# abiswas-odu/metagenomics

Measured on AMD Instinct MI355X. Metric: overlap edges/sec, higher is better.
Workload: dtype u64

## Files before the change

metagenomics_amd/csrc/device/mg_ctx.hpp:

```cpp
#ifndef MG_CTX_HPP_
#define MG_CTX_HPP_
#include <hip/hip_runtime.h>

#include <algorithm>
#include <cstdint>
#include <string>
#include <vector>

#include "mg_overlap.h"

__host__ __device__ constexpr int slot_words(int w) {
  return w <= 1 ? 1 : w <= 2 ? 2 : w <= 4 ? 4 : w <= 8 ? 8 : w <= 16 ? 16 : 32;
}

__host__ __device__ constexpr int slot_id_word(int w) { return slot_words(w) >= w + 2 ? slot_words(w) - 1 : -1; }
static_assert(slot_id_word(5) == 7 && slot_id_word(6) == 7 && slot_id_word(12) == 15, "widths with a spare word");
static_assert(slot_id_word(1) == -1 && slot_id_word(2) == -1 && slot_id_word(3) == -1 && slot_id_word(4) == -1 &&
                  slot_id_word(8) == -1 && slot_id_word(16) == -1 && slot_id_word(32) == -1,
              "widths whose slot ends at the pad word (or before it)");

template <typename T>
struct DevArray {
  T* p = nullptr;
  size_t cap = 0;
// ... 199 lines not shown
  uint8_t* xmarks = nullptr;
  uint64_t xchg_lo = 0, xchg_hi = 0;
  unsigned long long* d_blk = nullptr;
  size_t blk_cap = 0;
  unsigned long long* d_rcnt = nullptr;
  size_t rcnt_cap = 0;
  uint8_t* d_rdst = nullptr;
  size_t rdst_cap = 0;
  bool runs_meta8 = false;
  uint64_t super_zero_n = 0;
  unsigned long long* d_kblk = nullptr;
  size_t kblk_cap = 0;
  bool keys_counted = false;
  bool runs_counted = false;
  bool index_times_pending = false;
  unsigned long long* d_dcnt = nullptr;
  size_t dcnt_cap = 0;
  bool rows_counted = false;
  bool xchg_route_rows = true;
  bool xchg_scan_lds = true;
  uint32_t xchg_region = 512;
  uint32_t xchg_split_max = 4;
  int packable = 0;
  unsigned long long* d_flat_cnt = nullptr;
  size_t flat_cnt_cap = 0;
  unsigned long long* d_slot_cnt = nullptr;
  size_t slot_cnt_cap = 0;
  uint32_t* d_kb = nullptr;
  uint64_t* d_ke = nullptr;
  size_t kb_cap = 0, ke_cap = 0;
  hipEvent_t ev[16] = {};
  int scan_state = 0;
  bool runs_live = false;
  bool probe_share = true;
  bool probe_compact = true;
  uint64_t* d_key0 = nullptr;
  size_t key0_cap = 0;
  bool prefix_probe = true;
  ulonglong2* d_p0runs = nullptr;
  size_t p0runs_cap = 0;
  unsigned long long* d_p0cnt = nullptr;
  size_t p0cnt_cap = 0;
  uint32_t* d_xk[2] = {nullptr, nullptr};
  ulonglong2* d_xv[2] = {nullptr, nullptr};
  size_t xk_cap[2] = {0, 0}, xv_cap[2] = {0, 0};
  void* d_xsort_tmp = nullptr;
  size_t xsort_tmp_cap = 0;
  int xv_sel = 0;
  uint64_t xruns_n = 0;
  bool own_probed = false;
  bool xchg_keys_first = true;
  bool keys_first = false;
  bool rk_on = false;
  const uint64_t* rk_keys = nullptr;
  const unsigned long long* rk_cnt = nullptr;
  uint64_t rk_slot = 0, rk_total = 0;
  int xruns_part = 0;
  uint64_t xruns_K = 0;
  ulonglong2* d_xexp = nullptr;
  size_t xexp_cap = 0;
  bool xruns_ready = false;
  ulonglong2* xruns_base = nullptr;
  unsigned long long* xruns_cnt = nullptr;
  uint64_t xruns_reg = 0, xruns_nreg = 0;
  uint32_t* d_xkk[2] = {nullptr, nullptr};
  uint64_t* d_xke[2] = {nullptr, nullptr};
// ... 152 lines not shown
```

metagenomics_amd/csrc/device/mg_kernels.hip:

```cpp
#include <hip/hip_runtime.h>

#include <hipcub/hipcub.hpp>

#include <algorithm>
#include <cmath>
#include <cstdint>
#include <cstring>
#include <string>
#include <vector>

#include "mg_ctx.hpp"
#include "mg_overlap.h"

#ifndef MG_SCAN_UNROLL
#define MG_SCAN_UNROLL 1
#endif

namespace {

constexpr int kWave = 64;
constexpr int kBlock = 256;
constexpr int kWavesPerBlock = kBlock / kWave;
constexpr int kSegs = 64;
constexpr uint32_t kFpBits = 9;

__device__ __forceinline__ uint64_t mix64(uint64_t x) {
  x ^= x >> 31;
  x *= 0x7fb5d329728ea185ULL;
  x ^= x >> 27;
  x *= 0x81dadef4bc2dd44dULL;
  x ^= x >> 33;
  return x;
}

__device__ __forceinline__ uint32_t order_key(uint64_t mm) {
  const uint32_t lo = (uint32_t)mm, hi = (uint32_t)(mm >> 32);
  uint32_t x = __umul24(lo, 0x9E3779u) + (hi ^ (lo >> 8));
  x ^= x >> 15;
  x = __umul24(x, 0xEBCA77u) + (x >> 8);
  x ^= x >> 13;
  return x & 0xFFFFFC00u;
}

__device__ __forceinline__ uint64_t rc_word(uint64_t x) {
  x = __builtin_bitreverse64(~x);
// ... 611 lines not shown
  uint32_t recv_P;
  uint8_t* run_dst;
};

__device__ __forceinline__ int key_seg(int o) { return o == 0 ? 0 : (o == 1 ? 3 : o - 1); }

__device__ __forceinline__ void wave_sync() {
  __builtin_amdgcn_fence(__ATOMIC_RELEASE, "wavefront");
  __builtin_amdgcn_wave_barrier();
  __builtin_amdgcn_fence(__ATOMIC_ACQUIRE, "wavefront");
}

__device__ __forceinline__ uint64_t run_meta(uint64_t a, int p, int jlo, int jhi) {
  return (a & 0xFFFFFFFFull) | ((uint64_t)p << 32) | ((uint64_t)jlo << 42) | ((uint64_t)jhi << 52);
}


template <int MAXW>
__device__ __forceinline__ uint64_t ext_reg(const uint64_t* rw, int pos) {
  const int wi = pos >> 5;
  uint64_t w0 = rw[0], w1 = rw[1];
#pragma unroll
  for (int k = 1; k <= MAXW; ++k) {
    w0 = wi == k ? rw[k] : w0;
    w1 = wi + 1 == k ? rw[k] : w1;
  }
  if (wi + 1 > MAXW) w1 = 0;
  return funnel(w0, w1, (pos & 31) << 1);
}

#ifndef MG_SCAN_WAVES_G
#define MG_SCAN_WAVES_G 6
#endif
template <int MAXW, bool INDEX, bool KEYREC = false, int G = 1, bool RECV = false>
__global__ __launch_bounds__(kBlock) __attribute__((amdgpu_waves_per_eu(G > 1 ? MG_SCAN_WAVES_G : 6))) void k_scan(ScanParams p) {
  extern __shared__ __attribute__((aligned(16))) uint64_t smem[];
  const int lane = threadIdx.x & 63, wv = threadIdx.x >> 6;
  const int h = p.h, m = p.m, w = p.w;
  uint32_t* s_keys = reinterpret_cast<uint32_t*>(smem) + (size_t)wv * (w + kScanKeyPad) * kWave + lane;
  const int msh = 64 - 2 * m;
  const uint64_t mmask = (m == 32) ? ~0ULL : ((1ULL << (2 * m)) - 1);
  const uint64_t ngroups = (p.a_hi - p.a_lo + kWave - 1) / kWave;
  const int wpb = (int)(blockDim.x >> 6);
  const uint64_t gw = (uint64_t)blockIdx.x * wpb + wv;
  const uint64_t nw = (uint64_t)gridDim.x * wpb;
  uint64_t* s_buf = reinterpret_cast<uint64_t*>(smem) + (size_t)wpb * (((w + kScanKeyPad) * kWave + 1) / 2) +
                    (size_t)wv * kScanBuf;
  s_keys[w * kWave] = 0xFFFFFFFFu;
  ulonglong2* const region = p.runs + gw * G * p.run_cap;
  const uint64_t nbmask = (1ULL << p.nb_log2) - 1;
  uint64_t cur[G] = {};
  uint32_t dcnt = 0;
  uint32_t nbuf = 0;

  auto put = [&](bool flag, uint64_t meta) {
    const uint64_t bal = __ballot(flag);
    uint32_t at = nbuf + lane_prefix(bal);
    __asm__ volatile("" : "+v"(at));
    s_buf[flag ? at : 2 * kWave + lane] = meta;
    nbuf += (uint32_t)__popcll(bal);
  };
  const uint64_t nwin = (ngroups + G - 1) / G;
  uint64_t r_at = 0, r_end = 0, r_per = 0;
  if constexpr (RECV) {
    const uint64_t nch = (p.recv_total + 63) / 64;
    const uint64_t ch0 = nch * gw / nw, ch1 = nch * (gw + 1) / nw;
    r_at = ch0 * 64;
    r_end = min(ch1 * 64, p.recv_total);
// ... 38 lines not shown
   if (G > 1 && __builtin_amdgcn_readfirstlane(lmin) != __builtin_amdgcn_readfirstlane(lmax)) {
#pragma unroll
     for (int k = 2; k <= G * kWave; k <<= 1) {
#pragma unroll
       for (int j = k >> 1; j > 0; j >>= 1) {
#pragma unroll
         for (int q = 0; q < G; ++q) {
           const int e = lane + kWave * q;
           const bool up = (e & k) == 0;
           if (j >= kWave) {
             const int q2 = q ^ (j / kWave);
             if (q < q2) {
               const uint32_t x = wk[q], y = wk[q2];
               const bool sw = up ? x > y : x < y;
               wk[q] = sw ? y : x;
               wk[q2] = sw ? x : y;
             }
           } else {
             const uint32_t o = (uint32_t)__shfl_xor((int)wk[q], j);
             const bool low = (e & j) == 0;
             wk[q] = (low == up) ? min(wk[q], o) : max(wk[q], o);
           }
         }
       }
     }
   }
   for (int q = 0; q < G; ++q) {
    uint32_t key = wk[0];
#pragma unroll
    for (int qq = 1; qq < G; ++qq) key = q == qq ? wk[qq] : key;
    const uint32_t wslot = key & 255u;
    const uint64_t a = A0 + wslot;
    const int n = (int)(0x7FFu - (key >> 8));
    const uint64_t own = G > 1 ? ((uint64_t)lane << 8) | wslot : a;
    const uint64_t* g = p.words + a * slot_words(MAXW);
    const int J = n - h - 1;
    const int tend = J >= 1 ? J + w - 1 : 0;
    const int tlast = (INDEX && tend) ? tend + 1 : tend;
    int tmax = tlast;
#pragma unroll
    for (int d = 32; d >= 1; d >>= 1) tmax = max(tmax, __shfl_xor(tmax, d));
    tmax = __builtin_amdgcn_readfirstlane(tmax);
    constexpr int kRw = MAXW + 1 <= slot_words(MAXW) ? MAXW + 1 : slot_words(MAXW);
    uint64_t rw[MAXW + 1];
    {
      const uint64_t* gs = a < p.a_hi ? g : p.words;
#pragma unroll
      for (int k = 0; k <= MAXW; ++k) rw[k] = k < kRw ? gs[k] : 0;
    }
    __builtin_amdgcn_s_waitcnt(kWaitVm0);
    auto word_at = [&](int idx) {
      uint64_t v = rw[0];
#pragma unroll
      for (int k = 1; k <= MAXW; ++k) v = idx == k ? rw[k] : v;
      return v;
    };
    auto flush = [&](uint32_t k) {
      wave_sync();
      bool flag = (uint32_t)lane < k;
      uint64_t v = 0, meta = 0;
      if (flag) meta = s_buf[lane];
      const uint32_t ws = G > 1 ? (uint32_t)meta & 255u : (uint32_t)meta - (uint32_t)A0;
      if (G > 1) meta = (meta & ~0xFFFFFFFFull) | (uint32_t)(A0 + ws);
      if constexpr (MAXW <= 8) {
        const int pos = (int)((meta >> 32) & 1023u), wi = pos >> 5;
        const int src = !flag ? lane : G > 1 ? (int)((uint32_t)s_buf[lane] >> 8 & 63u) : (int)ws;
        uint64_t w0 = 0, w1 = 0;
  #pragma unroll
        for (int kk = 0; kk <= MAXW; ++kk) {
          const uint32_t lo = (uint32_t)__builtin_amdgcn_ds_bpermute(src << 2, (int)(uint32_t)rw[kk]);
          const uint32_t hi = (uint32_t)__builtin_amdgcn_ds_bpermute(src << 2, (int)(uint32_t)(rw[kk] >> 32));
          const uint64_t x = ((uint64_t)hi << 32) | lo;
          w0 = wi == kk ? x : w0;
          w1 = wi + 1 == kk ? x : w1;
        }
        if (flag) {
          v = mix64(funnel(w0, w1, (pos & 31) << 1) >> msh);
          if (!INDEX || p.nranks > 1) flag = owned(v & nbmask, p.nb_log2, p.rank, p.nranks);
        }
      } else if (flag) {
        const uint64_t* g2 = p.words + (meta & 0xFFFFFFFFull) * slot_words(MAXW);
        const int pos = (int)((meta >> 32) & 1023u);
        v = mix64(funnel(g2[pos >> 5], g2[(pos >> 5) + 1], (pos & 31) << 1) >> msh);
        if (!INDEX || p.nranks > 1) flag = owned(v & nbmask, p.nb_log2, p.rank, p.nranks);
      }
      uint64_t at_rec = 0;
      uint32_t grp_rec = 0;
      if constexpr (G == 1) {
        const uint64_t bal = __ballot(flag);
        const uint64_t at = cur[0] + lane_prefix(bal);
        at_rec = at;
        if constexpr (RECV) {
          if (flag && at < p.run_cap) {
            reinterpret_cast<uint64_t*>(p.runs)[gw * p.run_cap + at] = meta;
            p.run_dst[gw * p.run_cap + at] = (uint8_t)(((v & nbmask) * p.dst_ranks) >> p.nb_log2);
          }
        } else {
#if defined(MG_DIAG_STORE_NEVER)
        if (flag && at < p.run_cap && v == 0x0123456789ABCDEFull) region[at] = make_ulonglong2(v, meta);
#elif !defined(MG_DIAG_NO_RUNSTORE)
        if (flag && at < p.run_cap) region[at] = make_ulonglong2(v, meta);
#endif
        }
        cur[0] += (uint64_t)__popcll(bal);
      } else {
#ifdef MG_DIAG_ONE_REGION
        const uint32_t grp = 0;
#else
        const uint32_t grp = ws >> 6;
#endif
        uint64_t at = 0;
#pragma unroll
        for (int j = 0; j < G; ++j) {
          const uint64_t bal = __ballot(flag && grp == (uint32_t)j);
          if (grp == (uint32_t)j) at = cur[j] + lane_prefix(bal);
          cur[j] += (uint64_t)__popcll(bal);
        }
        at_rec = at;
        grp_rec = grp;
#if defined(MG_DIAG_STORE_NEVER)
        if (flag && at < p.run_cap && v == 0x0123456789ABCDEFull) region[grp * p.run_cap + at] = make_ulonglong2(v, meta);
#elif !defined(MG_DIAG_NO_RUNSTORE)
        if (flag && at < p.run_cap) region[grp * p.run_cap + at] = make_ulonglong2(v, meta);
#endif
      }
      if constexpr (KEYREC || RECV) {
        if (p.dst_cnt) {
          const bool st = flag && at_rec < p.run_cap;
          const uint32_t d = st ? (uint32_t)(((v & nbmask) * p.dst_ranks) >> p.nb_log2) : 0u;
          for (uint32_t jj = 0; jj < (uint32_t)G; ++jj)
            for (uint32_t dd = 0; dd < p.dst_ranks; ++dd) {
              const uint32_t cc = (uint32_t)__popcll(__ballot(st && grp_rec == jj && d == dd));
              dcnt += (uint32_t)lane == jj * p.dst_ranks + dd ? cc : 0u;
            }
        }
      }
      const uint32_t rest = nbuf - k;
      const uint64_t m0 = (uint32_t)lane < rest ? s_buf[k + lane] : 0;
      const uint64_t m1 = (uint32_t)lane + kWave < rest ? s_buf[k + kWave + lane] : 0;
      wave_sync();
      if ((uint32_t)lane < rest) s_buf[lane] = m0;
      if ((uint32_t)lane + kWave < rest) s_buf[kWave + lane] = m1;
      nbuf = rest;
      wave_sync();
      __builtin_amdgcn_s_waitcnt(0xC07F);
    };
    uint64_t mm = 0;
    if (tend) mm = funnel(rw[0], rw[1], 2) >> msh;
    uint32_t kb0 = 0xFFFFFFFFu, kb1 = 0xFFFFFFFFu;
    if (INDEX && tend) kb0 = order_key(rw[0] >> msh);
    uint32_t pmin = 0xFFFFFFFFu;
    int last_pos = 0, jlo = 1;
    int u = 0;
    uint32_t sv_pf = s_keys[kWave];
    auto roll_and_advance = [&](uint32_t key, uint64_t cw, int sh) {
      s_keys[u * kWave] = key;
      mm = ((mm << 2) | ((cw >> sh) & 3u)) & mmask;
      if (++u == w) {
        uint32_t run = 0xFFFFFFFFu;
        for (int v0 = w - 1; v0 >= 0; v0 -= 8) {
          uint32_t x8[8];
#pragma unroll
          for (int k = 0; k < 8; ++k) x8[k] = v0 - k >= 0 ? s_keys[(v0 - k) * kWave] : 0xFFFFFFFFu;
#pragma unroll
          for (int k = 0; k < 8; ++k) {
            run = x8[k] < run ? x8[k] : run;
            if (v0 - k >= 0) s_keys[(v0 - k) * kWave] = run;
          }
        }
        u = 0;
        pmin = 0xFFFFFFFFu;
      }
      sv_pf = s_keys[(u + 1) * kWave];
    };
    auto step_first = [&](int t, uint64_t cw, int sh) {
      const uint32_t key = order_key(mm) | (uint32_t)t;
      pmin = min(pmin, key);
      if (INDEX && t == w - 1) kb0 = min(kb0, pmin);
      if (t == w) last_pos = (int)(min(sv_pf, pmin) & 1023u);
      roll_and_advance(key, cw, sh);
    };
    auto step = [&](int t, uint64_t cw, int sh) {
      const uint32_t key = order_key(mm) | (uint32_t)t;
      pmin = min(pmin, key);
      const uint32_t mn = min(sv_pf, pmin);
      const int pos = (int)(mn & 1023u);
      if (INDEX) kb1 = t == tlast ? mn - (uint32_t)(n - h) : kb1;
      const bool live = t <= tend;
      const bool emit = live && pos != last_pos;
      const uint64_t e_meta = run_meta(own, last_pos, jlo, t - w);
      jlo = emit ? t - w + 1 : jlo;
      last_pos = live ? pos : last_pos;
      roll_and_advance(key, cw, sh);
      put(emit, e_meta);
      if (nbuf >= (uint32_t)kWave) flush(kWave);
    };
    if constexpr (MAXW <= 8) {
#pragma unroll
      for (int k = 0; k < MAXW + (INDEX ? 1 : 0); ++k) {
        const int t0 = max(1, 32 * k - m), t1 = min(tmax, 32 * k + 31 - m);
        const int tf = min(t1, w);
        for (int t = t0, sh = 62 - 2 * ((t0 + m) & 31); t <= tf; ++t, sh -= 2) step_first(t, rw[k], sh);
        int t = max(t0, w + 1), sh = 62 - 2 * ((t + m) & 31);
        if (t <= t1) {
#if MG_SCAN_UNROLL == 2
          for (; t + 1 <= t1; t += 2, sh -= 4) {
            step(t, rw[k], sh);
            step(t + 1, rw[k], sh - 2);
          }
          if (t <= t1) step(t, rw[k], sh);
#else
          do {
            step(t, rw[k], sh);
            sh -= 2;
          } while (++t <= t1);
#endif
        }
      }
    } else {
      int cwi = __builtin_amdgcn_readfirstlane((1 + m) >> 5);
      uint64_t cw = word_at(cwi);
      for (int t = 1; t <= tmax; ++t) {
        const int sh = 62 - 2 * ((t + m) & 31);
        if (t <= w) step_first(t, cw, sh); else step(t, cw, sh);
        const int xu = __builtin_amdgcn_readfirstlane(t + m);
        if ((xu & 31) == 31) cw = word_at((xu + 1) >> 5);
      }
    }
    put(tend > 0, run_meta(own, last_pos, jlo, J));
    while (nbuf) flush(nbuf < (uint32_t)kWave ? nbuf : (uint32_t)kWave);
    if (INDEX && tend) {
      uint32_t kb2 = 0xFFFFFFFFu, kb3 = 0xFFFFFFFFu;
      const bool w32 = w <= 32;
      if (w32) {
        const uint64_t Aw = ext_reg<MAXW>(rw, n - h);
        uint64_t r3 = rc_word(funnel(rw[0], rw[1], 2 * (w - 1))) & mmask;
        uint64_t r2 = rc_word(ext_reg<MAXW>(rw, n - m)) & mmask;
        for (int i = 0; i < w; ++i) {
          kb3 = min(kb3, order_key(r3) | (uint32_t)i);
          kb2 = min(kb2, order_key(r2) | (uint32_t)i);
          const int t3 = w - 2 - i;
          if (t3 >= 0) {
            r3 = ((r3 << 2) | (3u - ((rw[0] >> (62 - 2 * t3)) & 3u))) & mmask;
            r2 = ((r2 << 2) | (3u - ((Aw >> (62 - 2 * t3)) & 3u))) & mmask;
          }
        }
      } else {
        const uint64_t* gk = p.words + a * slot_words(MAXW);
        for (int i = 0; i < w; ++i) {
          kb3 = min(kb3, order_key(rc_word(ext_slot<MAXW>(gk, w - 1 - i)) & mmask) | (uint32_t)i);
          kb2 = min(kb2, order_key(rc_word(ext_slot<MAXW>(gk, n - m - i)) & mmask) | (uint32_t)i);
        }
      }
      const uint64_t nbm = (1ULL << p.nb_log2) - 1;
      const uint32_t kb[4] = {kb0, kb1, kb2, kb3};
      const int i0 = (int)(kb0 & 1023u), i1 = (int)(kb1 & 1023u), i2 = (int)(kb2 & 1023u), i3 = (int)(kb3 & 1023u);
      const uint64_t f0 = w32 ? funnel(rw[0], rw[1], i0 << 1) : ext_reg<MAXW>(rw, i0);
      const uint64_t f3 = w32 ? funnel(rw[0], rw[1], (w - 1 - i3) << 1) : ext_reg<MAXW>(rw, w - 1 - i3);
      const uint64_t mb[4] = {f0 >> msh, ext_reg<MAXW>(rw, n - h + i1) >> msh,
                              rc_word(ext_reg<MAXW>(rw, n - m - i2)) & mmask, rc_word(f3) & mmask};
      uint64_t cb[4];
      unsigned long long ce[4];
#pragma unroll
      for (int o = 0; o < 4; ++o) {
        const uint64_t v = mix64(mb[o]);
        const unsigned long long e = make_entry(v, p.nb_log2, (int)(kb[o] & 1023u), o, (uint32_t)a, n);
#ifndef MG_DIAG_NO_KEY0
        if (o == 0 && p.key0) p.key0[a] = (v & ((1ULL << 50) - 1)) | ((uint64_t)(kb[0] & 1023u) << 54);
        if constexpr (G > 1 || kWinGroups == 1) {
          if (o == 0 && p.p0runs) p.p0runs[a] = make_ulonglong2(v, run_meta(a, (int)(kb[0] & 1023u), 0, 0));
        }
#endif
        if constexpr (KEYREC) {
          p.key_bk[key_seg(o) * p.key_n + a - p.key_lo] = (uint32_t)(v & nbm);
          p.key_ent[key_seg(o) * p.key_n + a - p.key_lo] = (o == 1 && p.skip_o1) ? kEmpty : e;
        }
        cb[o] = v & nbm;
        ce[o] = e;
      }
      if constexpr (!KEYREC) {
#pragma unroll
        for (int o = 0; o < 4; ++o)
          if ((o != 1 || !p.skip_o1) && (o != 3 || !p.skip_o3) && !p.no_insert && owned(cb[o], p.nb_log2, p.rank, p.nranks))
            cell_insert(p.cells, cb[o] - p.cell_lo, p.cell_n, ce[o]);
      }
    } else if (INDEX && a < p.a_hi) {
      if (p.key0) p.key0[a] = kEmpty;
      if constexpr (G > 1 || kWinGroups == 1) {
        if (p.p0runs) p.p0runs[a] = make_ulonglong2(0, kFlatHole);
      }
      if constexpr (KEYREC) {
        for (int o = 0; o < 4; ++o) {
          p.key_bk[key_seg(o) * p.key_n + a - p.key_lo] = 0;
          p.key_ent[key_seg(o) * p.key_n + a - p.key_lo] = kEmpty;
        }
      }
    }
   }
   if constexpr (RECV) recv_insert(r_per);
  }
  if constexpr (RECV) recv_insert(~0ull);
  uint64_t c = cur[0];
#pragma unroll
  for (int j = 1; j < G; ++j) c = lane == j ? cur[j] : c;
  if (lane < G) p.run_cnt[gw * G + lane] = c;
  if constexpr (KEYREC || RECV) {
    if (p.dst_cnt && (uint32_t)lane < (uint32_t)G * p.dst_ranks)
      p.dst_cnt[(gw * G + lane / p.dst_ranks) * p.dst_ranks + lane % p.dst_ranks] = dcnt;
  }
}

template <int MAXW, int RING = kStageRing, bool FROM_MEM = false>
struct RunStage {
  const ScanParams& p;
  uint64_t* s_buf;
  ulonglong2* region;
  int lane, msh;
  uint64_t nbmask;
  uint64_t cursor = 0;
  uint32_t head = 0, nbuf = 0;
  uint32_t dcnt = 0;

  __device__ RunStage(const ScanParams& pp, uint64_t* buf, ulonglong2* reg, int ln)
      : p(pp), s_buf(buf), region(reg), lane(ln), msh(64 - 2 * pp.m), nbmask((1ULL << pp.nb_log2) - 1) {}

  __device__ __forceinline__ void put(bool flag, uint64_t meta) {
    const uint64_t bal = __ballot(flag);
    if (flag) s_buf[(head + nbuf + lane_prefix(bal)) & (RING - 1)] = meta;
// ... 1580 lines not shown

template <int W>
struct LaunchIndex {
  static int run(mg_ctx* ctx, uint64_t* cells = nullptr, bool all_keys = false) {
    IndexParams p = index_params(ctx);
    if (cells) p.cells = cells;
    p.skip_o1 = (!all_keys && !ctx->index_o1) ? 1 : 0;
    if (ctx->index_keys) {
      const uint32_t grid = (uint32_t)std::max<uint64_t>(
          1, std::min<uint64_t>((ctx->n + kBlock - 1) / kBlock, (uint64_t)ctx->n_cu * 16));
      if (!ctx->n) return 0;
      hipLaunchKernelGGL((k_index_keys<W>), dim3(grid), dim3(kBlock), 0, ctx->stream, p);
      return hipGetLastError() == hipSuccess ? 0 : -1;
    }
    uint32_t grid = (uint32_t)((4 * ctx->n + kBlock - 1) / kBlock);
    const size_t lds = (size_t)(W + 1) * kBlock * sizeof(uint64_t);
    if (grid == 0) return 0;
    allow_lds(k_index_build<W>, lds);
    hipLaunchKernelGGL((k_index_build<W>), dim3(grid), dim3(kBlock), lds, ctx->stream, p);
    return hipGetLastError() == hipSuccess ? 0 : -1;
  }
};

template <typename K>
uint32_t resident_blocks(mg_ctx* ctx, K kernel, size_t lds, uint64_t want, int block = kBlock) {
  allow_lds(kernel, lds);
  int per_cu = 0;
  (void)hipOccupancyMaxActiveBlocksPerMultiprocessor(&per_cu, kernel, block, lds);
  const uint64_t resident = (uint64_t)std::max(1, per_cu) * (uint64_t)std::max(1, ctx->n_cu);
  return (uint32_t)std::max<uint64_t>(1, std::min<uint64_t>(std::min<uint64_t>(want, resident), ctx->max_blocks));
}

constexpr size_t kLdsPerCu = 160 * 1024;
inline size_t scan_lds_per_wave(uint32_t w) {
  return (((size_t)(w + kScanKeyPad) * kWave + 1) / 2 + kScanBuf) * sizeof(uint64_t);
}
inline uint32_t scan_wpb(uint32_t w) {
  for (uint32_t wpb = kWavesPerBlock; wpb >= 1; wpb >>= 1)
    if (wpb * scan_lds_per_wave(w) <= kLdsPerCu) return wpb;
  return 0;
}
inline bool scan_is_reg(const mg_ctx* ctx, bool index) {
  if (ctx->rk_on) return false;
  return ctx->w <= (uint32_t)kRegW &&
         (!index || (ctx->xchg && !ctx->xchg_scan_lds && !(ctx->xchg_windows && ctx->minlen != ctx->maxlen)));
}
inline int scan_windows(const mg_ctx* ctx, bool index) {
  return (index && ctx->minlen != ctx->maxlen && !scan_is_reg(ctx, index)) ? kWinGroups : 1;
}
inline uint32_t scan_block_waves(const mg_ctx* ctx, bool index) {
  return scan_is_reg(ctx, index) ? kWavesPerBlock : scan_wpb(ctx->w);
}
inline size_t scan_lds(const mg_ctx* ctx, bool index) {
  return scan_is_reg(ctx, index) ? (size_t)kWavesPerBlock * kStageRing * sizeof(uint64_t)
                                 : (size_t)scan_wpb(ctx->w) * scan_lds_per_wave(ctx->w);
}
template <int W>
uint32_t scan_resident(mg_ctx* ctx, bool index, uint64_t want) {
  const size_t lds = scan_lds(ctx, index);
  const int block = (int)scan_block_waves(ctx, index) * kWave;
  if (scan_is_reg(ctx, index))
    return index ? resident_blocks(ctx, k_scan_reg<W, true>, lds, want, block)
                 : resident_blocks(ctx, k_scan_reg<W, false>, lds, want, block);
  if (index && ctx->xchg)
    return scan_windows(ctx, index) > 1 ? resident_blocks(ctx, k_scan<W, true, true, kWinGroups>, lds, want, block)
                                        : resident_blocks(ctx, k_scan<W, true, true>, lds, want, block);
  if (ctx->rk_on) return resident_blocks(ctx, k_scan<W, false, false, 1, true>, lds, want, block);
  return index ? (scan_windows(ctx, index) > 1 ? resident_blocks(ctx, k_scan<W, true, false, kWinGroups>, lds, want, block)
                                                : resident_blocks(ctx, k_scan<W, true>, lds, want, block))
               : resident_blocks(ctx, k_scan<W, false>, lds, want, block);
}

struct DiscGeom {
  uint32_t grid = 0, sgrid = 0, kreg = 1;
  size_t lds_scan = 0, lds_probe = 0;
};

template <int W>
DiscGeom disc_geom(mg_ctx* ctx, bool contain, uint64_t nsrc) {
  DiscGeom g;
  const uint64_t ngroups = (nsrc + kWave - 1) / kWave;
  const uint64_t want = std::max<uint64_t>(1, (ngroups + kWavesPerBlock - 1) / kWavesPerBlock);
  g.lds_scan = scan_lds(ctx, false);
  g.lds_probe = (size_t)kWavesPerBlock * ProbeLds<W>::bytes;
  g.grid = contain ? resident_blocks(ctx, k_probe<W, true>, g.lds_probe, want)
                   : resident_blocks(ctx, k_probe<W, false>, g.lds_probe, want);
  const uint32_t scan_res = scan_resident<W>(ctx, false, ~0ull >> 1);
  g.kreg = (uint32_t)std::max<uint64_t>(1, std::min<uint64_t>(scan_res / g.grid, (want + g.grid - 1) / g.grid));
  g.sgrid = g.grid * g.kreg;
  return g;
}

uint32_t fp_sort_bits(uint32_t hb) {
  if (hb >= 32) return 0;
  return std::min<uint32_t>((hb + 7) / 8 * 8 - hb, kFpBits);
}

template <int W>
struct LaunchScan {
  static int run(mg_ctx* ctx, bool contain, uint64_t a_lo, uint64_t a_hi, uint32_t sgrid, bool filter,
                 hipStream_t stream = nullptr, bool no_super = false, bool index = false) {
    if (!stream) stream = ctx->stream;
    const uint32_t wpb = scan_block_waves(ctx, index);
    const uint64_t nw = (uint64_t)sgrid * wpb;
    const uint64_t ngroups = (a_hi - a_lo + kWave - 1) / kWave;
    const uint64_t G = scan_is_reg(ctx, index) ? 1 : (uint64_t)scan_windows(ctx, index);
    const uint64_t nreg = nw * G;
    ctx->nrun_reg = nreg;
    const uint64_t Jmax = ctx->maxlen > ctx->h + 1 ? ctx->maxlen - ctx->h - 1 : 1;
    const uint64_t mid = ((uint64_t)ctx->minlen + ctx->maxlen) / 2;
    const uint64_t J = mid > ctx->h + 1 ? mid - ctx->h - 1 : 1;
    const uint64_t per_read = std::min<uint64_t>(Jmax, 2 * (2 * J / (ctx->w + 1) + 2));
    const uint64_t groups_per_region = ((ngroups + G - 1) / G + nw - 1) / nw;
    uint64_t run_cap = std::max<uint64_t>(
        ctx->run_cap_need, ctx->run_cap_opt ? ctx->run_cap_opt : groups_per_region * kWave * per_read);
    if (run_cap * nreg > ctx->runs_cap) {
      if (ctx->d_runs) (void)hipFree(ctx->d_runs);
      ctx->d_runs = nullptr;
      ctx->runs_cap = 0;
      if (ctx_malloc(ctx, (void**)&ctx->d_runs, run_cap * nreg * sizeof(ulonglong2), "d_runs (run regions)")) return -1;
      ctx->runs_cap = run_cap * nreg;
    }
    if (!ctx->run_cap_opt) run_cap = ctx->runs_cap / std::max<uint64_t>(1, nreg);
    ctx->run_cap = run_cap;
    if (ctx->run_cnt_cap < nreg) {
      if (ctx->d_run_cnt) (void)hipFree(ctx->d_run_cnt);
      ctx->d_run_cnt = nullptr;
      ctx->run_cnt_cap = 0;
      if (ctx_malloc(ctx, (void**)&ctx->d_run_cnt, std::max<uint64_t>(1, nreg) * sizeof(unsigned long long), "d_run_cnt"))
        return -1;
      ctx->run_cnt_cap = nreg;
    }
// ... 23 lines not shown
      else
        sp.key0 = ctx->d_key0;
    }
    sp.skip_o1 = (index && !ctx->index_o1) ? 1 : 0;
    sp.skip_o3 = (index && !ctx->index_o3 && !ctx->xchg) ? 1 : 0;
    sp.no_insert = (index && ctx->phase_limit == 1) ? 1 : 0;
    const bool recv = ctx->rk_on;
    ctx->runs_meta8 = false;
    if ((index || recv) && ctx->xchg) ctx->runs_counted = false;
    if ((index || recv) && ctx->xchg && ctx->nranks > 1 && G * ctx->nranks <= (uint64_t)kWave) {
      MG_ENSURE(d_rcnt, rcnt_cap, nreg * ctx->nranks);
      sp.dst_cnt = ctx->d_rcnt;
      sp.dst_ranks = ctx->nranks;
      ctx->runs_counted = true;
    }
    if (index && ctx->xchg) {
      sp.key_bk = ctx->d_kb;
      sp.key_ent = ctx->d_ke;
      sp.key_n = a_hi - a_lo;
      sp.key_lo = a_lo;
    }
    (void)hipEventRecord(ctx->ev[6], stream);
    if (scan_is_reg(ctx, index)) {
      if (index) {
        allow_lds(k_scan_reg<W, true>, lds);
        hipLaunchKernelGGL((k_scan_reg<W, true>), dim3(sgrid), dim3(wpb * kWave), lds, stream, sp);
        if (a_hi > a_lo)
          hipLaunchKernelGGL((k_rc_keys<W>), dim3((uint32_t)((a_hi - a_lo + kBlock - 1) / kBlock)), dim3(kBlock), 0,
                             stream, sp);
      } else {
        allow_lds(k_scan_reg<W, false>, lds);
        hipLaunchKernelGGL((k_scan_reg<W, false>), dim3(sgrid), dim3(wpb * kWave), lds, stream, sp);
      }
    } else if (index && ctx->xchg && G > 1) {
      allow_lds(k_scan<W, true, true, kWinGroups>, lds);
      hipLaunchKernelGGL((k_scan<W, true, true, kWinGroups>), dim3(sgrid), dim3(wpb * kWave), lds, stream, sp);
    } else if (index && ctx->xchg) {
      allow_lds(k_scan<W, true, true>, lds);
      hipLaunchKernelGGL((k_scan<W, true, true>), dim3(sgrid), dim3(wpb * kWave), lds, stream, sp);
    } else if (recv) {
      MG_ENSURE(d_rdst, rdst_cap, run_cap * nreg);
      sp.run_dst = ctx->d_rdst;
      ctx->runs_meta8 = true;
      sp.recv_keys = ctx->rk_keys;
      sp.recv_cnt = ctx->rk_cnt;
      sp.recv_slot = ctx->rk_slot;
      sp.recv_total = ctx->rk_total;
      sp.recv_P = ctx->nranks;
      sp.cell_lo = ctx->cell_lo;
      allow_lds(k_scan<W, false, false, 1, true>, lds);
      hipLaunchKernelGGL((k_scan<W, false, false, 1, true>), dim3(sgrid), dim3(wpb * kWave), lds, stream, sp);
    } else if (index && G > 1) {
      allow_lds(k_scan<W, true, false, kWinGroups>, lds);
      hipLaunchKernelGGL((k_scan<W, true, false, kWinGroups>), dim3(sgrid), dim3(wpb * kWave), lds, stream, sp);
    } else if (index) {
      allow_lds(k_scan<W, true>, lds);
      hipLaunchKernelGGL((k_scan<W, true>), dim3(sgrid), dim3(wpb * kWave), lds, stream, sp);
    } else {
      allow_lds(k_scan<W, false>, lds);
      hipLaunchKernelGGL((k_scan<W, false>), dim3(sgrid), dim3(wpb * kWave), lds, stream, sp);
    }
    (void)hipEventRecord(ctx->ev[7], stream);
    return hipGetLastError() == hipSuccess ? 0 : -1;
  }
};

int settle_rows(mg_ctx* ctx, bool* again);
int settle_runs(mg_ctx* ctx, bool* again);
int zero_stats(mg_ctx* ctx);

template <int W>
struct LaunchProbe {
  static int run(mg_ctx* ctx, bool contain, const ulonglong2* runs, const unsigned long long* run_cnt,
                 uint64_t run_cap, uint64_t run_regions, uint32_t grid, const uint32_t* src_super = nullptr,
                 uint64_t src_lo = 0, uint64_t src_hi = 0, bool append = false) {
    if (!contain && !ctx->index_o3 && !ctx->live_ready)
      return set_err(ctx, "discovery probe: the full index leaves out the o = 3 keys and no live index was built");
    if (ctx->maxlen > 1024)
      return set_err(ctx, "templated probe: reads longer than 1,024 bp must take the long-read kernels");
    ctx->nreg = (uint64_t)grid * kWavesPerBlock;
    ProbeParams pp{};
    pp.words = ctx->d_words;
    pp.len = ctx->d_len;
    pp.h = (int)ctx->h;
    pp.m = (int)ctx->m;
    pp.nb_log2 = ctx->nb_log2;
    pp.rank = ctx->rank;
    pp.nranks = ctx->nranks;
    pp.cell_lo = ctx->cell_lo;
    pp.cell_n = ctx->cell_n;
    pp.cells = ctx->d_cells;
    if (!contain && ctx->live_ready && ctx->live_coarse) {
      pp.cell_shift = ctx->live_shift;
// ... 541 lines not shown
  if (!strcmp(name, "xchg_keys_first")) {
    ctx->xchg_keys_first = value != 0;
    return 0;
  }
  if (!strcmp(name, "xchg_split_max")) {
    ctx->xchg_split_max = (uint32_t)std::max<int64_t>(0, value);
    return 0;
  }
  if (!strcmp(name, "xchg_region")) {
    if (value < 0 || value > 65536 || (value & (value - 1))) return set_err(ctx, "xchg_region: a power of two <= 65536");
    ctx->xchg_region = (uint32_t)value;
    return 0;
  }
  if (!strcmp(name, "alloc_cap")) {
    ctx->alloc_cap = (uint64_t)std::max<int64_t>(0, value);
    return 0;
  }
  if (!strcmp(name, "disc_block_cap")) {
    ctx->disc.block_cap = (uint32_t)std::max<int64_t>(0, std::min<int64_t>(value, 1 << 20));
    return 0;
  }
  if (!strcmp(name, "cov_budget")) {
    ctx->places.cov_budget = (uint64_t)std::max<int64_t>(0, value);
    return 0;
  }
  if (!strcmp(name, "run_cap")) {
    ctx->run_cap_opt = (uint64_t)std::max<int64_t>(0, value);
    ctx->run_cap_need = 0;
    return 0;
  }
  if (flag("stats", &ctx->stats) || flag("halving", &ctx->halving_low) || flag("layout", &ctx->layout) ||
      flag("contain_jcut", &ctx->contain_jcut) || flag("contain_skip", &ctx->contain_skip) ||
      flag("contain_prune", &ctx->contain_prune) || flag("cells_double", &ctx->cells_double) || flag("probe_share", &ctx->probe_share) ||
      flag("probe_compact", &ctx->probe_compact) || flag("live_index", &ctx->live_index) ||
      flag("xchg_sort_runs", &ctx->xchg_sort_runs) || flag("layout_scratch", &ctx->layout_scratch) ||
      flag("xchg_windows", &ctx->xchg_windows) || flag("chain_par", &ctx->chain_par) ||
      flag("live_runs", &ctx->live_runs) || flag("live_overlap", &ctx->live_overlap) ||
      flag("xchg_route_rows", &ctx->xchg_route_rows) || flag("xchg_scan_lds", &ctx->xchg_scan_lds))
    return 0;
  if (flag("prefix_contain", &ctx->prefix_contain) || flag("prefix_probe", &ctx->prefix_probe)) {
    ctx->index_ready = false;
    return 0;
  }
  return set_err(ctx, std::string("unknown option ") + name);
}

int mg_set_shard(mg_ctx* ctx, uint32_t rank, uint32_t nranks, uint64_t read_lo, uint64_t read_hi) {
  if (!ctx) return -1;
  if (nranks == 0 || rank >= nranks) return set_err(ctx, "bad shard rank/nranks");
  if (read_hi && read_hi < read_lo) return set_err(ctx, "bad read range");
  if (rank != ctx->rank || nranks != ctx->nranks || read_lo != ctx->read_lo || read_hi != ctx->read_hi) {
    ctx->index_ready = false;
    ctx->xchg = false;
    ctx->xchg_fused = false;
    ctx->xmarks_done = false;
    ctx->xmarks = nullptr;
    ctx->packable = 0;
  }
  ctx->rank = rank;
  ctx->nranks = nranks;
  ctx->read_lo = read_lo;
  ctx->read_hi = read_hi;
  return 0;
}

}
// ... 1545 lines not shown
```

Before: 18.47 billion.

## Record minimizer positions as per-read bitmasks and decode runs after the scan

Adds a mask variant of the scan kernel. Instead of buffering run candidates in LDS and flushing them through lane permutes, each lane marks its window-minimizer positions in a register bitmask, then pops the set bits to rebuild run boundaries and store them. This removes the per-wave LDS run buffer and the shuffle-heavy flush, which may raise occupancy. In exchange it adds register pressure, extra per-step work, a decode loop whose trip count follows the busiest lane, and more template instantiations. It is enabled by default when the read width is at most 8 words and the window is at most 32.

```diff
diff --git a/metagenomics_amd/csrc/device/mg_ctx.hpp b/metagenomics_amd/csrc/device/mg_ctx.hpp
--- a/metagenomics_amd/csrc/device/mg_ctx.hpp
+++ b/metagenomics_amd/csrc/device/mg_ctx.hpp
@@ -255,6 +255,7 @@
   hipEvent_t ev[16] = {};
   int scan_state = 0;
   bool runs_live = false;
+  bool run_masks = true;
   bool probe_share = true;
   bool probe_compact = true;
   uint64_t* d_key0 = nullptr;
diff --git a/metagenomics_amd/csrc/device/mg_kernels.hip b/metagenomics_amd/csrc/device/mg_kernels.hip
--- a/metagenomics_amd/csrc/device/mg_kernels.hip
+++ b/metagenomics_amd/csrc/device/mg_kernels.hip
@@ -11,6 +11,7 @@
 
 #include "mg_ctx.hpp"
 #include "mg_overlap.h"
+#include "mg_runs.hpp"
 
 #ifndef MG_SCAN_UNROLL
 #define MG_SCAN_UNROLL 1
@@ -688,8 +689,10 @@
 #ifndef MG_SCAN_WAVES_G
 #define MG_SCAN_WAVES_G 6
 #endif
-template <int MAXW, bool INDEX, bool KEYREC = false, int G = 1, bool RECV = false>
+constexpr int kMaskW = 32;
+template <int MAXW, bool INDEX, bool KEYREC = false, int G = 1, bool RECV = false, bool MASKS = false>
 __global__ __launch_bounds__(kBlock) __attribute__((amdgpu_waves_per_eu(G > 1 ? MG_SCAN_WAVES_G : 6))) void k_scan(ScanParams p) {
+  static_assert(!MASKS || MAXW <= 8, "the mask path keeps a read's words and both bit sets in registers");
   extern __shared__ __attribute__((aligned(16))) uint64_t smem[];
   const int lane = threadIdx.x & 63, wv = threadIdx.x >> 6;
   const int h = p.h, m = p.m, w = p.w;
@@ -794,7 +797,7 @@
     const uint32_t wslot = key & 255u;
     const uint64_t a = A0 + wslot;
     const int n = (int)(0x7FFu - (key >> 8));
-    const uint64_t own = G > 1 ? ((uint64_t)lane << 8) | wslot : a;
+    const uint64_t own = (G > 1 && !MASKS) ? ((uint64_t)lane << 8) | wslot : a;
     const uint64_t* g = p.words + a * slot_words(MAXW);
     const int J = n - h - 1;
     const int tend = J >= 1 ? J + w - 1 : 0;
@@ -803,6 +806,13 @@
 #pragma unroll
     for (int d = 32; d >= 1; d >>= 1) tmax = max(tmax, __shfl_xor(tmax, d));
     tmax = __builtin_amdgcn_readfirstlane(tmax);
+    int tall = 0;
+    if constexpr (MASKS) {
+      tall = tend ? tend : 0x7FFFFFFF;
+#pragma unroll
+      for (int d = 32; d >= 1; d >>= 1) tall = min(tall, __shfl_xor(tall, d));
+      tall = __builtin_amdgcn_readfirstlane(tall);
+    }
     constexpr int kRw = MAXW + 1 <= slot_words(MAXW) ? MAXW + 1 : slot_words(MAXW);
     uint64_t rw[MAXW + 1];
     {
@@ -816,6 +826,59 @@
 #pragma unroll
       for (int k = 1; k <= MAXW; ++k) v = idx == k ? rw[k] : v;
       return v;
+    };
+    auto store_run = [&](bool flag, uint64_t v, uint64_t meta, uint32_t grp_in) {
+      uint64_t at_rec = 0;
+      uint32_t grp_rec = 0;
+      if constexpr (G == 1) {
+        const uint64_t bal = __ballot(flag);
+        const uint64_t at = cur[0] + lane_prefix(bal);
+        at_rec = at;
+        if constexpr (RECV) {
+          if (flag && at < p.run_cap) {
+            reinterpret_cast<uint64_t*>(p.runs)[gw * p.run_cap + at] = meta;
+            p.run_dst[gw * p.run_cap + at] = (uint8_t)(((v & nbmask) * p.dst_ranks) >> p.nb_log2);
+          }
+        } else {
+#if defined(MG_DIAG_STORE_NEVER)
+        if (flag && at < p.run_cap && v == 0x0123456789ABCDEFull) region[at] = make_ulonglong2(v, meta);
+#elif !defined(MG_DIAG_NO_RUNSTORE)
+        if (flag && at < p.run_cap) region[at] = make_ulonglong2(v, meta);
+#endif
+        }
+        cur[0] += (uint64_t)__popcll(bal);
+      } else {
+#ifdef MG_DIAG_ONE_REGION
+        const uint32_t grp = 0;
+#else
+        const uint32_t grp = grp_in;
+#endif
+        uint64_t at = 0;
+#pragma unroll
+        for (int j = 0; j < G; ++j) {
+          const uint64_t bal = __ballot(flag && grp == (uint32_t)j);
+          if (grp == (uint32_t)j) at = cur[j] + lane_prefix(bal);
+          cur[j] += (uint64_t)__popcll(bal);
+        }
+        at_rec = at;
+        grp_rec = grp;
+#if defined(MG_DIAG_STORE_NEVER)
+        if (flag && at < p.run_cap && v == 0x0123456789ABCDEFull) region[grp * p.run_cap + at] = make_ulonglong2(v, meta);
+#elif !defined(MG_DIAG_NO_RUNSTORE)
+        if (flag && at < p.run_cap) region[grp * p.run_cap + at] = make_ulonglong2(v, meta);
+#endif
+      }
+      if constexpr (KEYREC || RECV) {
+        if (p.dst_cnt) {
+          const bool st = flag && at_rec < p.run_cap;
+          const uint32_t d = st ? (uint32_t)(((v & nbmask) * p.dst_ranks) >> p.nb_log2) : 0u;
+          for (uint32_t jj = 0; jj < (uint32_t)G; ++jj)
+            for (uint32_t dd = 0; dd < p.dst_ranks; ++dd) {
+              const uint32_t cc = (uint32_t)__popcll(__ballot(st && grp_rec == jj && d == dd));
+              dcnt += (uint32_t)lane == jj * p.dst_ranks + dd ? cc : 0u;
+            }
+        }
+      }
     };
     auto flush = [&](uint32_t k) {
       wave_sync();
@@ -846,57 +909,7 @@
         v = mix64(funnel(g2[pos >> 5], g2[(pos >> 5) + 1], (pos & 31) << 1) >> msh);
         if (!INDEX || p.nranks > 1) flag = owned(v & nbmask, p.nb_log2, p.rank, p.nranks);
       }
-      uint64_t at_rec = 0;
-      uint32_t grp_rec = 0;
-      if constexpr (G == 1) {
-        const uint64_t bal = __ballot(flag);
-        const uint64_t at = cur[0] + lane_prefix(bal);
-        at_rec = at;
-        if constexpr (RECV) {
-          if (flag && at < p.run_cap) {
-            reinterpret_cast<uint64_t*>(p.runs)[gw * p.run_cap + at] = meta;
-            p.run_dst[gw * p.run_cap + at] = (uint8_t)(((v & nbmask) * p.dst_ranks) >> p.nb_log2);
-          }
-        } else {
-#if defined(MG_DIAG_STORE_NEVER)
-        if (flag && at < p.run_cap && v == 0x0123456789ABCDEFull) region[at] = make_ulonglong2(v, meta);
-#elif !defined(MG_DIAG_NO_RUNSTORE)
-        if (flag && at < p.run_cap) region[at] = make_ulonglong2(v, meta);
-#endif
-        }
-        cur[0] += (uint64_t)__popcll(bal);
-      } else {
-#ifdef MG_DIAG_ONE_REGION
-        const uint32_t grp = 0;
-#else
-        const uint32_t grp = ws >> 6;
-#endif
-        uint64_t at = 0;
-#pragma unroll
-        for (int j = 0; j < G; ++j) {
-          const uint64_t bal = __ballot(flag && grp == (uint32_t)j);
-          if (grp == (uint32_t)j) at = cur[j] + lane_prefix(bal);
-          cur[j] += (uint64_t)__popcll(bal);
-        }
-        at_rec = at;
-        grp_rec = grp;
-#if defined(MG_DIAG_STORE_NEVER)
-        if (flag && at < p.run_cap && v == 0x0123456789ABCDEFull) region[grp * p.run_cap + at] = make_ulonglong2(v, meta);
-#elif !defined(MG_DIAG_NO_RUNSTORE)
-        if (flag && at < p.run_cap) region[grp * p.run_cap + at] = make_ulonglong2(v, meta);
-#endif
-      }
-      if constexpr (KEYREC || RECV) {
-        if (p.dst_cnt) {
-          const bool st = flag && at_rec < p.run_cap;
-          const uint32_t d = st ? (uint32_t)(((v & nbmask) * p.dst_ranks) >> p.nb_log2) : 0u;
-          for (uint32_t jj = 0; jj < (uint32_t)G; ++jj)
-            for (uint32_t dd = 0; dd < p.dst_ranks; ++dd) {
-              const uint32_t cc = (uint32_t)__popcll(__ballot(st && grp_rec == jj && d == dd));
-              dcnt += (uint32_t)lane == jj * p.dst_ranks + dd ? cc : 0u;
-            }
-        }
-      }
+      store_run(flag, v, meta, ws >> 6);
       const uint32_t rest = nbuf - k;
       const uint64_t m0 = (uint32_t)lane < rest ? s_buf[k + lane] : 0;
       const uint64_t m1 = (uint32_t)lane + kWave < rest ? s_buf[k + kWave + lane] : 0;
@@ -913,6 +926,7 @@
     if (INDEX && tend) kb0 = order_key(rw[0] >> msh);
     uint32_t pmin = 0xFFFFFFFFu;
     int last_pos = 0, jlo = 1;
+    uint32_t last_mn = 0;
     int u = 0;
     uint32_t sv_pf = s_keys[kWave];
     auto roll_and_advance = [&](uint32_t key, uint64_t cw, int sh) {
@@ -935,11 +949,15 @@
       }
       sv_pf = s_keys[(u + 1) * kWave];
     };
-    auto step_first = [&](int t, uint64_t cw, int sh) {
+    auto step_first = [&](int t, uint64_t cw, int sh, uint32_t& plo, uint32_t& phi, int cadd) {
       const uint32_t key = order_key(mm) | (uint32_t)t;
       pmin = min(pmin, key);
       if (INDEX && t == w - 1) kb0 = min(kb0, pmin);
-      if (t == w) last_pos = (int)(min(sv_pf, pmin) & 1023u);
+      if (t == w) {
+        last_mn = min(sv_pf, pmin);
+        last_pos = (int)(last_mn & 1023u);
+        if constexpr (MASKS) mg_runs::mark(plo, phi, last_mn + (uint32_t)cadd);
+      }
       roll_and_advance(key, cw, sh);
     };
     auto step = [&](int t, uint64_t cw, int sh) {
@@ -957,14 +975,40 @@
       put(emit, e_meta);
       if (nbuf >= (uint32_t)kWave) flush(kWave);
     };
+    auto step_all = [&](int t, uint64_t cw, int sh, uint32_t& plo, uint32_t& phi, int cadd) {
+      const uint32_t key = order_key(mm) | (uint32_t)t;
+      pmin = min(pmin, key);
+      last_mn = min(sv_pf, pmin);
+      mg_runs::mark(plo, phi, last_mn + (uint32_t)cadd);
+      roll_and_advance(key, cw, sh);
+    };
+    auto step_m = [&](int t, uint64_t cw, int sh, uint32_t& plo, uint32_t& phi, int cadd) {
+      const uint32_t key = order_key(mm) | (uint32_t)t;
+      pmin = min(pmin, key);
+      const uint32_t mn = min(sv_pf, pmin);
+      if (INDEX) kb1 = t == tlast ? mn - (uint32_t)(n - h) : kb1;
+      last_mn = t <= tend ? mn : last_mn;
+      mg_runs::mark(plo, phi, last_mn + (uint32_t)cadd);
+      roll_and_advance(key, cw, sh);
+    };
+    constexpr int NC = MASKS ? MAXW : 1;
+    uint32_t Pc[NC] = {};
     if constexpr (MAXW <= 8) {
 #pragma unroll
       for (int k = 0; k < MAXW + (INDEX ? 1 : 0); ++k) {
         const int t0 = max(1, 32 * k - m), t1 = min(tmax, 32 * k + 31 - m);
         const int tf = min(t1, w);
-        for (int t = t0, sh = 62 - 2 * ((t0 + m) & 31); t <= tf; ++t, sh -= 2) step_first(t, rw[k], sh);
+        uint32_t spare_lo = 0, spare_hi = 0;
+        uint32_t& plo = (MASKS && k >= 1 && k - 1 < NC) ? Pc[k >= 1 && k - 1 < NC ? k - 1 : 0] : spare_lo;
+        uint32_t& phi = (MASKS && k < NC) ? Pc[k < NC ? k : 0] : spare_hi;
+        const int cadd = m + 32 - 32 * k;
+        for (int t = t0, sh = 62 - 2 * ((t0 + m) & 31); t <= tf; ++t, sh -= 2) step_first(t, rw[k], sh, plo, phi, cadd);
         int t = max(t0, w + 1), sh = 62 - 2 * ((t + m) & 31);
-        if (t <= t1) {
+        if constexpr (MASKS) {
+          const int tq = min(t1, tall);
+          for (; t <= tq; ++t, sh -= 2) step_all(t, rw[k], sh, plo, phi, cadd);
+          for (; t <= t1; ++t, sh -= 2) step_m(t, rw[k], sh, plo, phi, cadd);
+        } else if (t <= t1) {
 #if MG_SCAN_UNROLL == 2
           for (; t + 1 <= t1; t += 2, sh -= 4) {
             step(t, rw[k], sh);
@@ -984,13 +1028,16 @@
       uint64_t cw = word_at(cwi);
       for (int t = 1; t <= tmax; ++t) {
         const int sh = 62 - 2 * ((t + m) & 31);
-        if (t <= w) step_first(t, cw, sh); else step(t, cw, sh);
+        uint32_t spare = 0;
+        if (t <= w) step_first(t, cw, sh, spare, spare, 0); else step(t, cw, sh);
         const int xu = __builtin_amdgcn_readfirstlane(t + m);
         if ((xu & 31) == 31) cw = word_at((xu + 1) >> 5);
       }
     }
-    put(tend > 0, run_meta(own, last_pos, jlo, J));
-    while (nbuf) flush(nbuf < (uint32_t)kWave ? nbuf : (uint32_t)kWave);
+    if constexpr (!MASKS) {
+      put(tend > 0, run_meta(own, last_pos, jlo, J));
+      while (nbuf) flush(nbuf < (uint32_t)kWave ? nbuf : (uint32_t)kWave);
+    }
     if (INDEX && tend) {
       uint32_t kb2 = 0xFFFFFFFFu, kb3 = 0xFFFFFFFFu;
       const bool w32 = w <= 32;
@@ -1056,6 +1103,47 @@
           p.key_bk[key_seg(o) * p.key_n + a - p.key_lo] = 0;
           p.key_ent[key_seg(o) * p.key_n + a - p.key_lo] = kEmpty;
         }
+      }
+    }
+    if constexpr (MASKS) {
+      mg_runs::clip<NC>(Pc, (int)(last_mn & 1023u) + m, tend > 0);
+      const uint32_t cnt = mg_runs::count<NC>(Pc);
+      int trips = (int)cnt;
+#pragma unroll
+      for (int d = 32; d >= 1; d >>= 1) trips = max(trips, __shfl_xor(trips, d));
+      trips = __builtin_amdgcn_readfirstlane(trips);
+      uint64_t R[MAXW + 1];
+      R[0] = 0;
+#pragma unroll
+      for (int k = 0; k < MAXW; ++k) R[k + 1] = rw[k];
+      auto carry = [&](bool sft) {
+#pragma unroll
+        for (int k = 0; k < MAXW; ++k) R[k] = sft ? R[k + 1] : R[k];
+      };
+      int xb = 0, jl = 1;
+#pragma unroll
+      for (int e = 0; e < 2; ++e) mg_runs::shift<NC>(Pc, xb, carry);
+      auto take = [&](int& rp, uint64_t& rm, uint32_t& rk) {
+        const int x = mg_runs::pop<NC, 0>(Pc, xb, carry);
+        rp = x - m;
+        rm = funnel(R[0], R[1], (x & 31) << 1) & mmask;
+        rk = order_key(rm) | (uint32_t)rp;
+      };
+      int pc, pn;
+      uint64_t mc, mnx;
+      uint32_t kc, kn;
+      take(pc, mc, kc);
+      for (int i = 0; i < trips; ++i) {
+        take(pn, mnx, kn);
+        bool flag = (uint32_t)i < cnt;
+        const int jh = mg_runs::run_end(pc, kc, pn, kn, (uint32_t)i + 1 >= cnt, J, w);
+        const uint64_t v = mix64(mc);
+        if (!INDEX || p.nranks > 1) flag = flag && owned(v & nbmask, p.nb_log2, p.rank, p.nranks);
+        store_run(flag, v, run_meta(a, pc, jl, jh), wslot >> 6);
+        jl = jh + 1;
+        pc = pn;
+        mc = mnx;
+        kc = kn;
       }
     }
    }
@@ -2702,13 +2790,16 @@
 }
 
 constexpr size_t kLdsPerCu = 160 * 1024;
-inline size_t scan_lds_per_wave(uint32_t w) {
-  return (((size_t)(w + kScanKeyPad) * kWave + 1) / 2 + kScanBuf) * sizeof(uint64_t);
-}
-inline uint32_t scan_wpb(uint32_t w) {
+inline size_t scan_lds_per_wave(uint32_t w, bool masks = false) {
+  return (((size_t)(w + kScanKeyPad) * kWave + 1) / 2 + (masks ? 0 : kScanBuf)) * sizeof(uint64_t);
+}
+inline uint32_t scan_wpb(uint32_t w, bool masks = false) {
   for (uint32_t wpb = kWavesPerBlock; wpb >= 1; wpb >>= 1)
-    if (wpb * scan_lds_per_wave(w) <= kLdsPerCu) return wpb;
+    if (wpb * scan_lds_per_wave(w, masks) <= kLdsPerCu) return wpb;
   return 0;
+}
+inline bool scan_masks(const mg_ctx* ctx) {
+  return ctx->run_masks && ctx->maxw <= 8 && ctx->w <= (uint32_t)kMaskW;
 }
 inline bool scan_is_reg(const mg_ctx* ctx, bool index) {
   if (ctx->rk_on) return false;
@@ -2719,11 +2810,21 @@
   return (index && ctx->minlen != ctx->maxlen && !scan_is_reg(ctx, index)) ? kWinGroups : 1;
 }
 inline uint32_t scan_block_waves(const mg_ctx* ctx, bool index) {
-  return scan_is_reg(ctx, index) ? kWavesPerBlock : scan_wpb(ctx->w);
+  return scan_is_reg(ctx, index) ? kWavesPerBlock : scan_wpb(ctx->w, scan_masks(ctx));
 }
 inline size_t scan_lds(const mg_ctx* ctx, bool index) {
   return scan_is_reg(ctx, index) ? (size_t)kWavesPerBlock * kStageRing * sizeof(uint64_t)
-                                 : (size_t)scan_wpb(ctx->w) * scan_lds_per_wave(ctx->w);
+                                 : (size_t)scan_wpb(ctx->w, scan_masks(ctx)) * scan_lds_per_wave(ctx->w, scan_masks(ctx));
+}
+template <int W, bool M>
+uint32_t scan_resident_k(mg_ctx* ctx, bool index, uint64_t want, size_t lds, int block) {
+  if (index && ctx->xchg)
+    return scan_windows(ctx, index) > 1 ? resident_blocks(ctx, k_scan<W, true, true, kWinGroups, false, M>, lds, want, block)
+                                        : resident_blocks(ctx, k_scan<W, true, true, 1, false, M>, lds, want, block);
+  if (ctx->rk_on) return resident_blocks(ctx, k_scan<W, false, false, 1, true, M>, lds, want, block);
+  return index ? (scan_windows(ctx, index) > 1 ? resident_blocks(ctx, k_scan<W, true, false, kWinGroups, false, M>, lds, want, block)
+                                                : resident_blocks(ctx, k_scan<W, true, false, 1, false, M>, lds, want, block))
+               : resident_blocks(ctx, k_scan<W, false, false, 1, false, M>, lds, want, block);
 }
 template <int W>
 uint32_t scan_resident(mg_ctx* ctx, bool index, uint64_t want) {
@@ -2732,13 +2833,10 @@
   if (scan_is_reg(ctx, index))
     return index ? resident_blocks(ctx, k_scan_reg<W, true>, lds, want, block)
                  : resident_blocks(ctx, k_scan_reg<W, false>, lds, want, block);
-  if (index && ctx->xchg)
-    return scan_windows(ctx, index) > 1 ? resident_blocks(ctx, k_scan<W, true, true, kWinGroups>, lds, want, block)
-                                        : resident_blocks(ctx, k_scan<W, true, true>, lds, want, block);
-  if (ctx->rk_on) return resident_blocks(ctx, k_scan<W, false, false, 1, true>, lds, want, block);
-  return index ? (scan_windows(ctx, index) > 1 ? resident_blocks(ctx, k_scan<W, true, false, kWinGroups>, lds, want, block)
-                                                : resident_blocks(ctx, k_scan<W, true>, lds, want, block))
-               : resident_blocks(ctx, k_scan<W, false>, lds, want, block);
+  if constexpr (W <= 8) {
+    if (scan_masks(ctx)) return scan_resident_k<W, true>(ctx, index, want, lds, block);
+  }
+  return scan_resident_k<W, false>(ctx, index, want, lds, block);
 }
 
 struct DiscGeom {
@@ -2768,6 +2866,30 @@
 
 template <int W>
 struct LaunchScan {
+  template <bool M>
+  static void launch_k(mg_ctx* ctx, bool index, bool recv, bool windows, uint32_t sgrid, uint32_t wpb, size_t lds,
+                       hipStream_t stream, const ScanParams& sp) {
+    const dim3 grid(sgrid), block(wpb * kWave);
+    if (index && ctx->xchg && windows) {
+      allow_lds(k_scan<W, true, true, kWinGroups, false, M>, lds);
+      hipLaunchKernelGGL((k_scan<W, true, true, kWinGroups, false, M>), grid, block, lds, stream, sp);
+    } else if (index && ctx->xchg) {
+      allow_lds(k_scan<W, true, true, 1, false, M>, lds);
+      hipLaunchKernelGGL((k_scan<W, true, true, 1, false, M>), grid, block, lds, stream, sp);
+    } else if (recv) {
+      allow_lds(k_scan<W, false, false, 1, true, M>, lds);
+      hipLaunchKernelGGL((k_scan<W, false, false, 1, true, M>), grid, block, lds, stream, sp);
+    } else if (index && windows) {
+      allow_lds(k_scan<W, true, false, kWinGroups, false, M>, lds);
+      hipLaunchKernelGGL((k_scan<W, true, false, kWinGroups, false, M>), grid, block, lds, stream, sp);
+    } else if (index) {
+      allow_lds(k_scan<W, true, false, 1, false, M>, lds);
+      hipLaunchKernelGGL((k_scan<W, true, false, 1, false, M>), grid, block, lds, stream, sp);
+    } else {
+      allow_lds(k_scan<W, false, false, 1, false, M>, lds);
+      hipLaunchKernelGGL((k_scan<W, false, false, 1, false, M>), grid, block, lds, stream, sp);
+    }
+  }
   static int run(mg_ctx* ctx, bool contain, uint64_t a_lo, uint64_t a_hi, uint32_t sgrid, bool filter,
                  hipStream_t stream = nullptr, bool no_super = false, bool index = false) {
     if (!stream) stream = ctx->stream;
@@ -2857,33 +2979,24 @@
         allow_lds(k_scan_reg<W, false>, lds);
         hipLaunchKernelGGL((k_scan_reg<W, false>), dim3(sgrid), dim3(wpb * kWave), lds, stream, sp);
       }
-    } else if (index && ctx->xchg && G > 1) {
-      allow_lds(k_scan<W, true, true, kWinGroups>, lds);
-      hipLaunchKernelGGL((k_scan<W, true, true, kWinGroups>), dim3(sgrid), dim3(wpb * kWave), lds, stream, sp);
-    } else if (index && ctx->xchg) {
-      allow_lds(k_scan<W, true, true>, lds);
-      hipLaunchKernelGGL((k_scan<W, true, true>), dim3(sgrid), dim3(wpb * kWave), lds, stream, sp);
-    } else if (recv) {
-      MG_ENSURE(d_rdst, rdst_cap, run_cap * nreg);
-      sp.run_dst = ctx->d_rdst;
-      ctx->runs_meta8 = true;
-      sp.recv_keys = ctx->rk_keys;
-      sp.recv_cnt = ctx->rk_cnt;
-      sp.recv_slot = ctx->rk_slot;
-      sp.recv_total = ctx->rk_total;
-      sp.recv_P = ctx->nranks;
-      sp.cell_lo = ctx->cell_lo;
-      allow_lds(k_scan<W, false, false, 1, true>, lds);
-      hipLaunchKernelGGL((k_scan<W, false, false, 1, true>), dim3(sgrid), dim3(wpb * kWave), lds, stream, sp);
-    } else if (index && G > 1) {
-      allow_lds(k_scan<W, true, false, kWinGroups>, lds);
-      hipLaunchKernelGGL((k_scan<W, true, false, kWinGroups>), dim3(sgrid), dim3(wpb * kWave), lds, stream, sp);
-    } else if (index) {
-      allow_lds(k_scan<W, true>, lds);
-      hipLaunchKernelGGL((k_scan<W, true>), dim3(sgrid), dim3(wpb * kWave), lds, stream, sp);
     } else {
-      allow_lds(k_scan<W, false>, lds);
-      hipLaunchKernelGGL((k_scan<W, false>), dim3(sgrid), dim3(wpb * kWave), lds, stream, sp);
+      if (recv) {
+        MG_ENSURE(d_rdst, rdst_cap, run_cap * nreg);
+        sp.run_dst = ctx->d_rdst;
+        ctx->runs_meta8 = true;
+        sp.recv_keys = ctx->rk_keys;
+        sp.recv_cnt = ctx->rk_cnt;
+        sp.recv_slot = ctx->rk_slot;
+        sp.recv_total = ctx->rk_total;
+        sp.recv_P = ctx->nranks;
+        sp.cell_lo = ctx->cell_lo;
+      }
+      bool masks = false;
+      if constexpr (W <= 8) masks = scan_masks(ctx);
+      if constexpr (W <= 8) {
+        if (masks) launch_k<true>(ctx, index, recv, G > 1, sgrid, wpb, lds, stream, sp);
+      }
+      if (!masks) launch_k<false>(ctx, index, recv, G > 1, sgrid, wpb, lds, stream, sp);
     }
     (void)hipEventRecord(ctx->ev[7], stream);
     return hipGetLastError() == hipSuccess ? 0 : -1;
@@ -3491,6 +3604,7 @@
   if (flag("stats", &ctx->stats) || flag("halving", &ctx->halving_low) || flag("layout", &ctx->layout) ||
       flag("contain_jcut", &ctx->contain_jcut) || flag("contain_skip", &ctx->contain_skip) ||
       flag("contain_prune", &ctx->contain_prune) || flag("cells_double", &ctx->cells_double) || flag("probe_share", &ctx->probe_share) ||
+      flag("run_masks", &ctx->run_masks) ||
       flag("probe_compact", &ctx->probe_compact) || flag("live_index", &ctx->live_index) ||
       flag("xchg_sort_runs", &ctx->xchg_sort_runs) || flag("layout_scratch", &ctx->layout_scratch) ||
       flag("xchg_windows", &ctx->xchg_windows) || flag("chain_par", &ctx->chain_par) ||
diff --git a/metagenomics_amd/csrc/device/mg_runs.hpp b/metagenomics_amd/csrc/device/mg_runs.hpp
--- /dev/null
+++ b/metagenomics_amd/csrc/device/mg_runs.hpp
@@ -0,0 +1,83 @@
+#pragma once
+#include <cstdint>
+
+#if defined(__HIPCC__)
+#define MG_RUNS_HD __host__ __device__ __forceinline__
+#else
+#define MG_RUNS_HD inline
+#endif
+
+namespace mg_runs {
+
+MG_RUNS_HD void mark(uint32_t& lo, uint32_t& hi, uint32_t s) {
+  const uint64_t b = 1ull << (s & 63u);
+  lo |= (uint32_t)b;
+  hi |= (uint32_t)(b >> 32);
+}
+
+template <int N>
+MG_RUNS_HD void clip(uint32_t (&c)[N], int X, bool valid) {
+  const int xc = X >> 5;
+  const uint32_t part = 0xFFFFFFFFu >> (31 - (X & 31));
+#pragma unroll
+  for (int k = 0; k < N; ++k) c[k] = (!valid || k > xc) ? 0u : (k == xc ? c[k] & part : c[k]);
+}
+
+template <int N>
+MG_RUNS_HD uint32_t count(const uint32_t (&c)[N]) {
+  uint32_t n = 0;
+#pragma unroll
+  for (int k = 0; k < N; ++k) n += (uint32_t)__builtin_popcount(c[k]);
+  return n;
+}
+
+template <int N, class F>
+MG_RUNS_HD void shift(uint32_t (&c)[N], int& base, F&& carry) {
+  const bool s = c[0] == 0;
+#pragma unroll
+  for (int k = 0; k + 1 < N; ++k) c[k] = s ? c[k + 1] : c[k];
+  c[N - 1] = s ? 0u : c[N - 1];
+  base += s ? 32 : 0;
+  carry(s);
+}
+
+template <int N, int EXTRA, class F>
+MG_RUNS_HD int pop(uint32_t (&c)[N], int& base, F&& carry) {
+#pragma unroll
+  for (int e = 0; e <= EXTRA; ++e) shift<N>(c, base, carry);
+  const uint32_t v = c[0];
+  const int b = __builtin_ctz(v | 0x80000000u);
+  c[0] = v & (v - 1u);
+  return base + b;
+}
+
+struct NoCarry {
+  MG_RUNS_HD void operator()(bool) const {}
+};
+
+MG_RUNS_HD int run_end(int p, uint32_t key, int pn, uint32_t keyn, bool last, int J, int w) {
+  return last ? J : (keyn < key ? pn - w : p);
+}
+
+template <int N, class K>
+MG_RUNS_HD bool decode(const uint32_t (&P0)[N], int J, int m, int w, uint32_t i, K&& key_at, int& p, int& lo, int& hi) {
+  uint32_t P[N];
+  for (int k = 0; k < N; ++k) P[k] = P0[k];
+  const uint32_t n = count<N>(P);
+  if (i >= n) return false;
+  int xb = 0;
+  int pc = pop<N, N - 1>(P, xb, NoCarry()) - m;
+  lo = 1;
+  for (uint32_t r = 0;; ++r) {
+    const int pn = pop<N, N - 1>(P, xb, NoCarry()) - m;
+    const bool last = r + 1 == n;
+    hi = run_end(pc, key_at(pc), pn, last ? 0u : key_at(pn), last, J, w);
+    if (r == i) break;
+    lo = hi + 1;
+    pc = pn;
+  }
+  p = pc;
+  return true;
+}
+
+}
```

Measured after the change: 19.22 billion (median of 6 runs). 1.04x the previous value.
